# engcang/FAST-LIO-SAM-QN

Measured on AMD Instinct MI355X. Metric: scan-pair registrations/sec on 100k-pt clouds, higher is better.
Workload: dtype f32 search / f64 accumulate

## Files before the change

fast-lio-sam-qn_amd/csrc/qn_gicp_kernels.cuh:

```cuda
#pragma once
#include "qn_device.cuh"
#include "qn_step_math.cuh"
#include "qn_linearize.cuh"
#include "qn_knn_hist.cuh"
#include "../../include/qn_engine.h"
#include "qn_util_kernels.cuh"

namespace qn {

#define QN_ACC_MAX_BLOCKS 512
#define QN_MAX_TRACE 1024

struct GicpState {
  double x0[16], xi[16], delta[16];
  double H[36], b[6], d[6];
  double y0, yi, den;
  double lambda, nu;
  double final_H[36];
  double fitness;
  int outer, inner, phase, converged, lm_failed;
  uint32_t fb_count;
  uint32_t trace_len;
  uint32_t big_count;
  int pending;
  int reserved;
};


__device__ __forceinline__ uint32_t xcd_block(uint32_t b, uint32_t nb) {
  const uint32_t per = nb >> 3, rem = nb & 7u, x = b & 7u;
  return x * per + min(x, rem) + (b >> 3);
}

struct CellCountK {
  static constexpr int TB = QN_BLOCK, OCC = 1;
  struct Args { const float4* pts; uint32_t n; GridView g; uint32_t* counts; uint32_t* cell_of_pt; };
  static __device__ __forceinline__ void run(const Args& a, const uint32_t bx, const uint32_t) {
    const GridView g = grid_resolve(a.g);
    const uint32_t i = bx * QN_BLOCK + threadIdx.x;
    if (i >= a.n) return;
    const float4 p = a.pts[i];
    const int cx = cell_coord(p.x, g.ox, g.inv_cell, g.nx), cy = cell_coord(p.y, g.oy, g.inv_cell, g.ny), cz = cell_coord(p.z, g.oz, g.inv_cell, g.nz);
    const uint32_t c = cell_key(g, cx, cy, cz);
    a.cell_of_pt[i] = c;
    atomicAdd(&a.counts[c], 1u);
  }
};
static __global__ void __launch_bounds__(QN_BLOCK) k_cell_count(const float4* __restrict__ pts, uint32_t n, GridView g, uint32_t* __restrict__ counts, uint32_t* __restrict__ cell_of_pt) {
  const CellCountK::Args a{pts, n, g, counts, cell_of_pt};
  CellCountK::run(a, blockIdx.x, gridDim.x);
}

__device__ inline GridDims grid_dims_from_bbox(const int (&omn)[3], const int (&omx)[3], bool bad, uint32_t n, uint32_t max_cells, double cell_override) {
  GridDims d;
  float mn[3], mx[3];
  for (int a = 0; a < 3; a++) { mn[a] = ord2f(omn[a]); mx[a] = ord2f(omx[a]); }
  bad = bad || !(mx[0] >= mn[0]);
  if (bad) { for (int a = 0; a < 3; a++) { mn[a] = 0.f; mx[a] = 0.f; } }
  double L[3]; for (int a = 0; a < 3; a++) L[a] = fmax((double)mx[a] - (double)mn[a], 0.0);
  const double Lmax = fmax(L[0], fmax(L[1], L[2]));
  const double area = fmax(L[0] * L[1], fmax(L[0] * L[2], L[1] * L[2]));
  double cell = sqrt(4.0 * area / (double)n);
  cell = fmax(cell, fmax(Lmax / 2048.0, 1e-6));
  if (cell_override > 0) cell = cell_override;
  int dims[3] = {1, 1, 1}, tdims[3] = {1, 1, 1}; const int tile[3] = {QN_TX, QN_TY, QN_TZ};
  for (int iter = 0; iter < 64; iter++) {
    double tot = 1;
    for (int a = 0; a < 3; a++) { dims[a] = (int)floor(L[a] / cell) + 1; tdims[a] = (dims[a] + tile[a] - 1) / tile[a]; tot *= (double)tdims[a] * tile[a]; }
    if (tot <= (double)max_cells) break;
    cell *= fmax(cbrt(tot / (double)max_cells), 1.02);
    if (iter == 63) { cell = Lmax + 1.0; for (int a = 0; a < 3; a++) { dims[a] = 1; tdims[a] = 1; } }
  }
  d.ox = mn[0]; d.oy = mn[1]; d.oz = mn[2]; d.cell = (float)cell; d.inv_cell = 1.0f / d.cell;
  d.nx = dims[0]; d.ny = dims[1]; d.nz = dims[2]; d.ntx = tdims[0]; d.nty = tdims[1]; d.ntz = tdims[2];
  float amax = 0; for (int a = 0; a < 3; a++) amax = fmaxf(amax, fmaxf(fabsf(mn[a]), fabsf(mx[a])));
  d.eps = 1e-3f * d.cell + 1e-6f * (amax + (float)Lmax);
  d.n = bad ? 0u : n; d.ncells = (uint32_t)tdims[0] * tdims[1] * tdims[2] * QN_TILE_CELLS; d.nonfinite = bad ? 1u : 0u; d.pad = 0;
  return d;
}

#define QN_BBOX_MAX_BLOCKS 256
struct BBoxAcc { int mn[3], mx[3]; uint32_t nonfinite, ticket; };
struct PackBBoxK {
  static constexpr int TB = QN_BLOCK, OCC = 1;
  struct Args { const char* in; uint32_t stride, n; float4* raw; BBoxAcc* acc; uint32_t max_cells; double cell_override; GridDims* dims_dev; GridDims* dims_host; };
  static __device__ __forceinline__ void run(const Args& a, const uint32_t bx, const uint32_t nbx) {
    __shared__ int smn[QN_BLOCK / 64][3], smx[QN_BLOCK / 64][3], sbad[QN_BLOCK / 64];
    const char* __restrict__ in = a.in; float4* __restrict__ raw = a.raw; BBoxAcc* acc = a.acc;
    const uint32_t n = a.n, stride = a.stride;
    int mn[3] = {0x7fffffff, 0x7fffffff, 0x7fffffff}, mx[3] = {(int)0x80000000, (int)0x80000000, (int)0x80000000};
    int bad = 0;
    for (uint32_t i = bx * QN_BLOCK + threadIdx.x; i < n; i += nbx * QN_BLOCK) {
      const float* q = (const float*)(in + (size_t)i * stride);
      const float4 p = make_float4(q[0], q[1], q[2], 1.0f);
      raw[i] = p;
      if (!(isfinite(p.x) && isfinite(p.y) && isfinite(p.z))) { bad = 1; continue; }
      const int ox = f2ord(p.x), oy = f2ord(p.y), oz = f2ord(p.z);
      mn[0] = min(mn[0], ox); mn[1] = min(mn[1], oy); mn[2] = min(mn[2], oz);
      mx[0] = max(mx[0], ox); mx[1] = max(mx[1], oy); mx[2] = max(mx[2], oz);
    }
#pragma unroll
    for (int d = 0; d < 3; d++) { mn[d] = wave_min_i(mn[d]); mx[d] = wave_max_i(mx[d]); }
    bad = wave_max_i(bad);
    const int wid = threadIdx.x >> 6;
    if ((threadIdx.x & 63) == 0) { for (int d = 0; d < 3; d++) { smn[wid][d] = mn[d]; smx[wid][d] = mx[d]; } sbad[wid] = bad; }
    __syncthreads();
    __shared__ int s_last;
    if (threadIdx.x == 0) {
      for (int w = 1; w < QN_BLOCK / 64; w++) { for (int d = 0; d < 3; d++) { mn[d] = min(mn[d], smn[w][d]); mx[d] = max(mx[d], smx[w][d]); } bad |= sbad[w]; }
      BBoxAcc* mine = acc + 1 + bx;
      for (int d = 0; d < 3; d++) { __hip_atomic_store(&mine->mn[d], mn[d], __ATOMIC_RELAXED, __HIP_MEMORY_SCOPE_AGENT); __hip_atomic_store(&mine->mx[d], mx[d], __ATOMIC_RELAXED, __HIP_MEMORY_SCOPE_AGENT); }
      __hip_atomic_store(&mine->nonfinite, (uint32_t)bad, __ATOMIC_RELAXED, __HIP_MEMORY_SCOPE_AGENT);
      asm volatile("s_waitcnt vmcnt(0)" ::: "memory");
      s_last = __hip_atomic_fetch_add(&acc->ticket, 1u, __ATOMIC_RELAXED, __HIP_MEMORY_SCOPE_AGENT) == nbx - 1u ? 1 : 0;
    }
    __syncthreads();
    if (!s_last) return;
    if (threadIdx.x >= 64) return;
    for (int d = 0; d < 3; d++) { mn[d] = 0x7fffffff; mx[d] = (int)0x80000000; }
    int nf = 0;
    for (uint32_t b = threadIdx.x; b < nbx; b += 64) {
      const BBoxAcc* o = acc + 1 + b;
      for (int d = 0; d < 3; d++) { mn[d] = min(mn[d], __hip_atomic_load(&o->mn[d], __ATOMIC_RELAXED, __HIP_MEMORY_SCOPE_AGENT)); mx[d] = max(mx[d], __hip_atomic_load(&o->mx[d], __ATOMIC_RELAXED, __HIP_MEMORY_SCOPE_AGENT)); }
      nf |= (int)__hip_atomic_load(&o->nonfinite, __ATOMIC_RELAXED, __HIP_MEMORY_SCOPE_AGENT);
    }
#pragma unroll
    for (int d = 0; d < 3; d++) { mn[d] = wave_min_i(mn[d]); mx[d] = wave_max_i(mx[d]); }
    nf = wave_max_i(nf);
    if (threadIdx.x != 0) return;
    const GridDims g = grid_dims_from_bbox(mn, mx, nf != 0, n, a.max_cells, a.cell_override);
    *a.dims_dev = g; *a.dims_host = g;
    __hip_atomic_store(&acc->ticket, 0u, __ATOMIC_RELAXED, __HIP_MEMORY_SCOPE_AGENT);
  }
};
static __global__ void __launch_bounds__(QN_BLOCK) k_pack_bbox_dims(const char* __restrict__ in, uint32_t stride, uint32_t n, float4* __restrict__ raw, BBoxAcc* acc,
                                                                    uint32_t max_cells, double cell_override, GridDims* __restrict__ dims_dev, GridDims* __restrict__ dims_host) {
  const PackBBoxK::Args a{in, stride, n, raw, acc, max_cells, cell_override, dims_dev, dims_host};
  PackBBoxK::run(a, blockIdx.x, gridDim.x);
}
static __global__ void k_bbox_acc_init(BBoxAcc* acc, int count) {
  for (int i = threadIdx.x; blockIdx.x == 0 && i < count; i += blockDim.x) { BBoxAcc a; for (int d = 0; d < 3; d++) { a.mn[d] = 0x7fffffff; a.mx[d] = (int)0x80000000; } a.nonfinite = 0; a.ticket = 0; acc[i] = a; }
}

#define QN_LB_STATE_AGG 1ull
#define QN_LB_STATE_INC 2ull
struct ScanLookbackK {
  static constexpr int TB = QN_BLOCK, OCC = 1;
  struct Args { const uint32_t* in; const GridDims* dims; uint32_t* out; unsigned long long* status; uint32_t epoch, total; };
  static __device__ __forceinline__ void run(const Args& a, const uint32_t bx, const uint32_t) {
    __shared__ uint32_t wsum[QN_BLOCK / 64];
    __shared__ uint32_t s_prefix;
    const uint32_t* __restrict__ in = a.in; uint32_t* __restrict__ out = a.out; unsigned long long* status = a.status;
    const uint32_t total = a.total;
    const uint32_t m = uni(a.dims->ncells);
    const uint32_t tile = bx;
    if (tile * (uint32_t)(QN_BLOCK * QN_SCAN_ITEMS) >= m) return;
// ... 319 lines not shown
  using Args = NnSearchArgs;
  static __device__ __forceinline__ void run(const Args& a, const uint32_t bx, const uint32_t nbx) {
    GridView src = a.src, tgt = a.tgt; const GicpState* __restrict__ st = a.st; const double thr2 = a.thr2; float r0 = a.r0; const int max_rounds = a.max_rounds;
    int32_t* __restrict__ corr = a.corr; float* __restrict__ sqd = a.sqd; int32_t* __restrict__ nn_idx = a.nn_idx; float4* __restrict__ nn_ref = a.nn_ref;
    uint2* __restrict__ fb_list = a.fb_list; uint32_t* __restrict__ fb_count = a.fb_count; uint2* __restrict__ big_list = a.big_list; uint32_t* __restrict__ big_count = a.big_count;
    const int big_blocks = a.big_blocks; const float big_ratio = a.big_ratio; uint32_t* __restrict__ far_stats = a.far_stats; const NnOpt opt = a.opt;

  __shared__ WaveLds lds[BLOCK / 64];
  if (MODE == 0 && uni(st->phase) != 0) return;
  if (MODE == 1 && uni(st->phase) != 2) return;
  if (opt.cond && !(uni(st->reserved) & opt.cond)) return;
  src = grid_resolve(src); tgt = grid_resolve(tgt); if (r0 < 0.f) r0 = -r0 * tgt.cell;
  __shared__ float sTf[12];
  if (threadIdx.x < 12) sTf[threadIdx.x] = (float)st->x0[threadIdx.x];
  __syncthreads();
  if (LIST && (int)bx >= (int)nbx - big_blocks) {
    const uint32_t nbig = uni(*big_count);
    if (tgt.dbg && bx == nbx - 1 && threadIdx.x == 0) atomicAdd(&tgt.dbg[7], nbig);
    uint32_t nfar = 0;
    const uint32_t bw0 = (bx - (nbx - big_blocks)) * (BLOCK / 64) + (threadIdx.x >> 6), nbw = big_blocks * (BLOCK / 64);
    const uint32_t E = (GROUP && opt.group && nbig >= (uint32_t)opt.group_min) ? min(16u, (nbig + (uint32_t)opt.group - 1u) / (uint32_t)opt.group) : 1u;
    if (GROUP && E > 1u) {
      const int lane = threadIdx.x & 63, qs = lane & 15;
      WaveLds* wl = &lds[threadIdx.x >> 6];
      const float INF = __int_as_float(0x7f800000);
      for (uint32_t w0 = bw0 * E; w0 < nbig; w0 += nbw * E) {
        const uint32_t slot = w0 + (uint32_t)qs;
        const bool active = (uint32_t)qs < E && slot < nbig;
        const uint2 rec = active ? big_list[slot] : make_uint2(0u, 0u);
        const float4 p = active ? src.pts[rec.x] : make_float4(0.f, 0.f, 0.f, 0.f);
        float qx, qy, qz; { float Tf[12];
#pragma unroll
          for (int j = 0; j < 12; j++) Tf[j] = sTf[j];
          xform_query<MODE>(Tf, p.x, p.y, p.z, qx, qy, qz); }
        const float v = __uint_as_float(rec.y);
        const float r = v > 0.f ? v * 1.1f + 0.5f * tgt.cell : -v;
        const bool finite_q = (qx - qx == 0.f) && (qy - qy == 0.f) && (qz - qz == 0.f) && (r - r == 0.f);
        unsigned long long key = QN_INF_KEY; float second = INF, d_unseen = INF;
        unsigned long long todo = __ballot(active);
        while (todo) {
          const int al = __ffsll((long long)todo) - 1;
          const float ax = rdlane(qx, al), ay = rdlane(qy, al), az = rdlane(qz, al), ar = rdlane(r, al);
          const bool afin = rdlane((int)finite_q, al) != 0;
          const bool open_q = (todo >> lane) & 1ull;
          const bool member = open_q && (qs == (al & 15) || (afin && finite_q && sqdist(qx, qy, qz, ax, ay, az) <= 0.25f * ar * ar));
          const unsigned long long mm = __ballot(member);
          if (__popcll(mm) <= 4) {
            unsigned long long k1; float s1, du1;
            wave_search_single(tgt, ax, ay, az, ar, INF, k1, s1, du1, wl);
            if (member) { key = k1; second = s1; d_unseen = du1; }
          } else {
            wave_search_far16(tgt, qx, qy, qz, member, r, key, second, d_unseen, wl);
          }
          todo &= ~mm;
        }
        if (active && lane < 16) {
          const uint32_t tl = late(rec.x);
          store_nn<MODE>(key, late(__float_as_uint(p.w)), tl, thr2, corr, sqd, nn_idx);
          if (MODE == 0) nn_ref[tl] = make_float4(qx, qy, qz, key != QN_INF_KEY ? sqrtf(key_d2(key)) : INF);
        }
        if (far_stats && MODE == 0) {
          const unsigned long long fm = __ballot(active && lane < 16 && key != QN_INF_KEY && key_d2(key) > 36.f * tgt.cell * tgt.cell);
          if (lane == 0) nfar += (uint32_t)__popcll(fm);
        }
      }
      if (far_stats && MODE == 0 && (threadIdx.x & 63) == 0 && nfar) atomicAdd(&far_stats[3], nfar);
      return;
    }
    unsigned long long pr_sum = 0, pr_max = 0, pr_a = 0, pr_b = 0; uint32_t pr_n = 0;
    const uint32_t nfb_all = uni(*fb_count);
    const uint32_t nfb1 = (opt.fb_small && nfb_all <= opt.fb_small) ? nfb_all : 0u;
    for (uint32_t w = bw0; w < nbig + nfb1; w += nbw) {
      const uint2 rec = w < nbig ? big_list[w] : fb_list[w - nbig];
      const float4 p = src.pts[rec.x];
      float qx, qy, qz; { float Tf[12];
#pragma unroll
          for (int j = 0; j < 12; j++) Tf[j] = sTf[j];
          xform_query<MODE>(Tf, p.x, p.y, p.z, qx, qy, qz); }
      const float v = __uint_as_float(rec.y);
      const float r = v > 0.f ? v * 1.1f + 0.5f * tgt.cell : -v;
      unsigned long long key; float second, d_unseen;
      const unsigned long long pt0 = opt.probe ? wall_clock64() : 0ull;
      SingleStats sst;
      wave_search_single(tgt, qx, qy, qz, r, __int_as_float(0x7f800000), key, second, d_unseen, &lds[threadIdx.x >> 6], sst, opt.probe != nullptr);
      if (opt.probe) { const unsigned long long dt = wall_clock64() - pt0; pr_sum += dt; pr_n++;
        if (dt > pr_max) { pr_max = dt; pr_a = ((unsigned long long)sst.rounds << 48) | ((unsigned long long)min(sst.segs, 0xffffffu) << 24) | (unsigned long long)min(sst.cand, 0xffffffu);
          pr_b = ((unsigned long long)__float_as_uint(sst.r_first) << 32) | __float_as_uint(key != QN_INF_KEY ? sqrtf(key_d2(key)) : -1.f); } }
      if ((threadIdx.x & 63) == 0) {
        const uint32_t tl = late(rec.x);
        store_nn<MODE>(key, late(__float_as_uint(p.w)), tl, thr2, corr, sqd, nn_idx);
        if (MODE == 0) nn_ref[tl] = make_float4(qx, qy, qz, fminf(sqrtf(second), d_unseen));
        if (key != QN_INF_KEY && key_d2(key) > 36.f * tgt.cell * tgt.cell) nfar++;
      }
    }
    if (far_stats && MODE == 0 && (threadIdx.x & 63) == 0 && nfar) atomicAdd(&far_stats[3], nfar);
    if (opt.probe && (threadIdx.x & 63) == 0 && bw0 < 16384u) { opt.probe[4 * bw0] = (pr_max << 32) | pr_n; opt.probe[4 * bw0 + 1] = pr_sum; opt.probe[4 * bw0 + 2] = pr_a; opt.probe[4 * bw0 + 3] = pr_b; }
    return;
  }
  const uint32_t nq = LIST ? uni(*fb_count) : src.n;
  if (LIST && opt.fb_small && nq <= opt.fb_small) return;
  if (LIST && tgt.dbg && bx == 0 && threadIdx.x == 0) atomicAdd(&tgt.dbg[5], nq);
  const uint32_t wave0 = bx * (BLOCK / 64) + (threadIdx.x >> 6), nwaves = (nbx - (LIST ? big_blocks : 0)) * (BLOCK / 64);
  for (uint32_t base = wave0 * 16; base < nq; base += nwaves * 16) {
    const uint32_t slot = base + (threadIdx.x & 15);
    const bool active = slot < nq;
    uint32_t t = slot; float r = r0, r_cap = __int_as_float(0x7f800000);
    if (LIST && active) {
      const uint2 rec = fb_list[slot]; t = rec.x;
      const float v = __uint_as_float(rec.y);
      if (v < 0.f) r = -v; else { r_cap = v; r = fminf(v, r0); }
    }
    const float4 p = active ? src.pts[t] : make_float4(0, 0, 0, 0);
    float qx, qy, qz; { float Tf[12];
#pragma unroll
          for (int j = 0; j < 12; j++) Tf[j] = sTf[j];
          xform_query<MODE>(Tf, p.x, p.y, p.z, qx, qy, qz); }
    Best1 sink; sink.init();
    float d_unseen;
    const bool cert = wave_search<4>(tgt, qx, qy, qz, active, r, r_cap, max_rounds, sink, &lds[threadIdx.x >> 6], d_unseen);
    const bool mine = active && (threadIdx.x & 48) == 0;
    const bool done = cert || LIST;
    if (!LIST && MODE == 0 && opt.clear_ref && mine) opt.clear_ref[t] = make_float4(0.f, 0.f, 0.f, 0.f);
    if (mine && done) {
      const uint32_t tl = late(t);
      store_nn<MODE>(sink.key, late(__float_as_uint(p.w)), tl, thr2, corr, sqd, nn_idx);
      if (MODE == 0) nn_ref[tl] = make_float4(qx, qy, qz, fminf(sqrtf(sink.second), d_unseen));
    }
    if (!LIST) {
      const float rn = r;
      const bool far = rn > big_ratio * r0;
      wave_append(big_list, big_count, mine && !done && far, make_uint2(t, __float_as_uint(-rn)));
      wave_append(fb_list, fb_count, mine && !done && !far, make_uint2(t, __float_as_uint(-rn)));
    }
  }
  }
};
template <int MODE, bool LIST, int BLOCK, bool GROUP = false>
__global__ void __launch_bounds__(BLOCK, GROUP ? 5 : 6) k_nn_search(GridView src, GridView tgt, const GicpState* __restrict__ st, double thr2, float r0, int max_rounds,
                                                        int32_t* __restrict__ corr, float* __restrict__ sqd, int32_t* __restrict__ nn_idx, float4* __restrict__ nn_ref,
                                                        uint2* __restrict__ fb_list, uint32_t* __restrict__ fb_count,
                                                        uint2* __restrict__ big_list, uint32_t* __restrict__ big_count, int big_blocks, float big_ratio, uint32_t* __restrict__ far_stats, NnOpt opt) {
  const NnSearchArgs a{src, tgt, st, thr2, r0, max_rounds, corr, sqd, nn_idx, nn_ref, fb_list, fb_count, big_list, big_count, big_blocks, big_ratio, far_stats, opt};
  NnSearchK<MODE, LIST, BLOCK, GROUP>::run(a, blockIdx.x, gridDim.x);
}


typedef __attribute__((address_space(1))) unsigned long long qn_gu64;
__device__ __forceinline__ void pr_store(unsigned long long* p, unsigned long long bits) { __hip_atomic_store((qn_gu64*)p, bits, __ATOMIC_RELAXED, __HIP_MEMORY_SCOPE_AGENT); }
__device__ __forceinline__ unsigned long long pr_load(const unsigned long long* p) { return __hip_atomic_load((qn_gu64*)p, __ATOMIC_RELAXED, __HIP_MEMORY_SCOPE_AGENT); }
__device__ __forceinline__ void row_store(double* p, double v, const bool coherent) {
  if (coherent) pr_store((unsigned long long*)p, (unsigned long long)__double_as_longlong(v)); else *p = v;
}

#define QN_LANE_ROWS 9
template <int MODE>
struct NnLaneK {
  static constexpr int TB = 256, OCC = 6;
  using Args = NnSearchArgs;
  static __device__ __forceinline__ void run(const Args& a, const uint32_t bx, const uint32_t) {
    const GicpState* __restrict__ st = a.st; const NnOpt opt = a.opt;
    if (MODE == 0 && uni(st->phase) != 0) return;
    if (MODE == 1 && uni(st->phase) != 2) return;
    if (opt.cond && !(uni(st->reserved) & opt.cond)) return;
    const GridView src = grid_resolve(a.src), tgt = grid_resolve(a.tgt);
    float r0 = a.r0; if (r0 < 0.f) r0 = -r0 * tgt.cell;
    float Tf[12];
#pragma unroll
    for (int j = 0; j < 12; j++) Tf[j] = uni((float)st->x0[j]);
    const uint32_t t = bx * TB + threadIdx.x;
    const bool active = t < src.n;
    const float4 p = active ? src.pts[t] : make_float4(0, 0, 0, 0);
    float qx, qy, qz; xform_query<MODE>(Tf, p.x, p.y, p.z, qx, qy, qz);
    if (MODE == 0 && opt.clear_ref && active) opt.clear_ref[t] = make_float4(0.f, 0.f, 0.f, 0.f);
    float r = r0;
    const int x0 = cell_coord(qx - r, tgt.ox, tgt.inv_cell, tgt.nx), x1 = cell_coord(qx + r, tgt.ox, tgt.inv_cell, tgt.nx);
    const int y0 = cell_coord(qy - r, tgt.oy, tgt.inv_cell, tgt.ny), y1 = cell_coord(qy + r, tgt.oy, tgt.inv_cell, tgt.ny);
    const int z0 = cell_coord(qz - r, tgt.oz, tgt.inv_cell, tgt.nz), z1 = cell_coord(qz + r, tgt.oz, tgt.inv_cell, tgt.nz);
    const int tx0 = x0 >> 3, ntr = (x1 >> 3) - tx0 + 1, nyr = y1 - y0 + 1, nzr = z1 - z0 + 1;
    const bool scan = active && nyr <= 3 && nzr <= 3 && ntr <= 2;
    Best1 sink; sink.init();
    const float4* __restrict__ pts = tgt.pts; const uint32_t* __restrict__ cs = tgt.cell_start;
    const uint32_t tile_zy = (uint32_t)tgt.nty * (uint32_t)tgt.ntx;
    uint32_t kz[3], ky[3];
#pragma unroll
    for (int d = 0; d < 3; d++) {
      const int z = z0 + d, y = y0 + d;
      kz[d] = (((uint32_t)(z >> 2) * tile_zy) << 7) | ((uint32_t)(z & 3) << 5);
      ky[d] = (((uint32_t)(y >> 2) * (uint32_t)tgt.ntx) << 7) | ((uint32_t)(y & 3) << 3);
    }
    const bool two = scan && ntr == 2;
    const int xb0 = min(x1, (tx0 << 3) + 7);
    const uint32_t kx0 = ((uint32_t)tx0 << 7) | (uint32_t)(x0 & 7), xlen0 = (uint32_t)(xb0 - x0) + 1u;
    const uint32_t kx1 = (uint32_t)(tx0 + 1) << 7, xlen1 = (uint32_t)(x1 - ((tx0 + 1) << 3)) + 1u;
    uint32_t s0[QN_LANE_ROWS], len0[QN_LANE_ROWS], off1[QN_LANE_ROWS], tot[QN_LANE_ROWS];
#pragma unroll
    for (int rr = 0; rr < QN_LANE_ROWS; rr++) {
      const int dz = rr / 3, dy = rr % 3;
      const bool rv = scan && dy < nyr && dz < nzr;
      uint32_t a0 = 0, b0 = 0, a1 = 0, b1 = 0;
      const uint32_t kr = kz[dz] + ky[dy];
      if (rv) { a0 = cs[kr + kx0]; b0 = cs[kr + kx0 + xlen0]; }
      if (rv && two) { a1 = cs[kr + kx1]; b1 = cs[kr + kx1 + xlen1]; }
      s0[rr] = a0; len0[rr] = b0 - a0; off1[rr] = a1 - len0[rr]; tot[rr] = len0[rr] + (b1 - a1);
    }
#pragma unroll
    for (int rr = 0; rr < QN_LANE_ROWS; rr++) {
      const uint32_t l0 = len0[rr], sa = s0[rr], sb = off1[rr], last = tot[rr] - 1u;
      for (uint32_t v = 0; v < tot[rr]; v += 4) {
        const uint32_t v1 = min(v + 1u, last), v2 = min(v + 2u, last), v3 = min(v + 3u, last);
        const float4 c0 = pts[v + (v < l0 ? sa : sb)], c1 = pts[v1 + (v1 < l0 ? sa : sb)], c2 = pts[v2 + (v2 < l0 ? sa : sb)], c3 = pts[v3 + (v3 < l0 ? sa : sb)];
        sink.consider<true>(true, sqdist(qx, qy, qz, c0.x, c0.y, c0.z), __float_as_uint(c0.w));
        sink.consider<true>(v + 1u <= last, sqdist(qx, qy, qz, c1.x, c1.y, c1.z), __float_as_uint(c1.w));
        sink.consider<true>(v + 2u <= last, sqdist(qx, qy, qz, c2.x, c2.y, c2.z), __float_as_uint(c2.w));
        sink.consider<true>(v + 3u <= last, sqdist(qx, qy, qz, c3.x, c3.y, c3.z), __float_as_uint(c3.w));
      }
    }
    const float INF = __int_as_float(0x7f800000);
    bool certified = false; float d_unseen = INF;
    if (scan) {
      float d = INF;
      if (x0 > 0) d = fminf(d, qx - (tgt.ox + x0 * tgt.cell));
      if (x1 < tgt.nx - 1) d = fminf(d, (tgt.ox + (x1 + 1) * tgt.cell) - qx);
      if (y0 > 0) d = fminf(d, qy - (tgt.oy + y0 * tgt.cell));
      if (y1 < tgt.ny - 1) d = fminf(d, (tgt.oy + (y1 + 1) * tgt.cell) - qy);
      if (z0 > 0) d = fminf(d, qz - (tgt.oz + z0 * tgt.cell));
      if (z1 < tgt.nz - 1) d = fminf(d, (tgt.oz + (z1 + 1) * tgt.cell) - qz);
      if (d == INF || !(r == r)) { certified = true; d_unseen = INF; }
      else { d -= tgt.eps; d_unseen = d; certified = d > 0.f && sink.full() && sink.worst_d2() < d * d; }
      if (!certified) r = sink.full() ? fmaxf(sqrtf(sink.worst_d2()) * 1.000001f + tgt.eps, r + tgt.eps) : 2.f * r + tgt.cell;
    }
    if (active && certified) {
      store_nn<MODE>(sink.key, __float_as_uint(p.w), t, a.thr2, a.corr, a.sqd, a.nn_idx);
      if (MODE == 0) a.nn_ref[t] = make_float4(qx, qy, qz, fminf(sqrtf(sink.second), d_unseen));
    }
    const bool far = r > a.big_ratio * r0;
    wave_append(a.big_list, a.big_count, active && !certified && far, make_uint2(t, __float_as_uint(-r)));
    wave_append(a.fb_list, a.fb_count, active && !certified && !far, make_uint2(t, __float_as_uint(-r)));
  }
};
template <int MODE>
__global__ void __launch_bounds__(256, 6) k_nn_lane(NnSearchArgs a) { NnLaneK<MODE>::run(a, blockIdx.x, gridDim.x); }


#define QN_TRACK_SEG 8
__device__ __forceinline__ bool track_bound_holds(float d0, float delta, float bound) {
  return (sqrtf(d0) + delta) * 1.000004f < bound;
}
template <int MODE>
__global__ void __launch_bounds__(QN_BLOCK, 6) k_nn_track(GridView src, GridView tgt, const float4* __restrict__ tgt_raw, const GicpState* __restrict__ st,
                                                       double thr2, int32_t* __restrict__ corr, float* __restrict__ sqd, int32_t* __restrict__ nn_idx,
                                                       float4* __restrict__ nn_ref, uint2* __restrict__ fb_list, uint32_t* __restrict__ fb_count,
                                                       uint2* __restrict__ big_list, uint32_t* __restrict__ big_count) {
  if (MODE == 0 && st->phase != 0) return;
  if (MODE == 1 && st->phase != 2) return;
  src = grid_resolve(src); tgt = grid_resolve(tgt);
  float Tf[12];
#pragma unroll
  for (int j = 0; j < 12; j++) Tf[j] = (float)st->x0[j];
  const uint32_t lblk = xcd_block(blockIdx.x, gridDim.x);
  const uint32_t t = lblk * QN_BLOCK + threadIdx.x;
  if (t >= src.n) return;
  const float INF = __int_as_float(0x7f800000);
  const float4 p = src.pts[t];
  const uint32_t i = __float_as_uint(p.w);
  float qx, qy, qz; xform_query<MODE>(Tf, p.x, p.y, p.z, qx, qy, qz);
  unsigned long long best = QN_INF_KEY; float second = INF, d_unseen = INF;
  bool rescanned = false, big = false, noseed = false;
  float r = 0.f, delta = 0.f;
  const bool finite_q = (qx - qx == 0.f) && (qy - qy == 0.f) && (qz - qz == 0.f);
  const uint32_t j0 = (uint32_t)nn_idx[t];
  if (finite_q && j0 >= tgt.n) { noseed = true; big = true; r = tgt.cell; }
  if (finite_q && !noseed) {
    const float4 ref = nn_ref[t];
    const float4 p0 = tgt_raw[j0];
    const float d0 = sqdist(qx, qy, qz, p0.x, p0.y, p0.z);
    best = pack_key(d0, j0);
    delta = sqrtf(sqdist(qx, qy, qz, ref.x, ref.y, ref.z));
    if (track_bound_holds(d0, delta, ref.w)) {
      if (tgt.dbg && (threadIdx.x & 63) == 0) atomicAdd(&tgt.dbg[6], (uint32_t)__popcll(__ballot(1)));
    } else {
      r = sqrtf(d0) * 1.000001f + tgt.eps;
      const int bx0 = cell_coord(qx - r, tgt.ox, tgt.inv_cell, tgt.nx), bx1 = cell_coord(qx + r, tgt.ox, tgt.inv_cell, tgt.nx);
      const int by0 = cell_coord(qy - r, tgt.oy, tgt.inv_cell, tgt.ny), by1 = cell_coord(qy + r, tgt.oy, tgt.inv_cell, tgt.ny);
      const int bz0 = cell_coord(qz - r, tgt.oz, tgt.inv_cell, tgt.nz), bz1 = cell_coord(qz + r, tgt.oz, tgt.inv_cell, tgt.nz);
      const int tx0 = bx0 >> 3, ntr = (bx1 >> 3) - tx0 + 1, nyr = by1 - by0 + 1;
      const int nseg = ntr * nyr * (bz1 - bz0 + 1);
      if (!(d0 == d0) || nseg > QN_TRACK_SEG) big = true;
      else {
        uint32_t s[QN_TRACK_SEG], e[QN_TRACK_SEG];
#pragma unroll
        for (int sg = 0; sg < QN_TRACK_SEG; sg++) {
          s[sg] = 0; e[sg] = 0;
          if (sg < nseg) {
            int tt, rr; divmod_small(sg, ntr, rr, tt);
            int qz_, ry_; divmod_small(rr, nyr, qz_, ry_);
            const int ry = by0 + ry_, rz = bz0 + qz_, tx = tx0 + tt;
            const int xa = max(bx0, tx << 3), xb = min(bx1, (tx << 3) + 7);
            const uint32_t k0 = cell_key(tgt, xa, ry, rz);
            s[sg] = tgt.cell_start[k0]; e[sg] = tgt.cell_start[k0 + (xb - xa) + 1];
          }
        }
#pragma unroll
        for (int sg = 0; sg < QN_TRACK_SEG; sg++) {
          for (uint32_t u = s[sg]; u < e[sg]; u++) {
            const float4 a = tgt.pts[u];
            const float da = sqdist(qx, qy, qz, a.x, a.y, a.z);
            const unsigned long long ka = pack_key(da, __float_as_uint(a.w));
            if (ka < best) { second = key_d2(best); best = ka; }
            else if (ka != best && da < second) second = da;
          }
        }
        float d = INF;
        if (bx0 > 0) d = fminf(d, qx - (tgt.ox + bx0 * tgt.cell));
        if (bx1 < tgt.nx - 1) d = fminf(d, (tgt.ox + (bx1 + 1) * tgt.cell) - qx);
        if (by0 > 0) d = fminf(d, qy - (tgt.oy + by0 * tgt.cell));
        if (by1 < tgt.ny - 1) d = fminf(d, (tgt.oy + (by1 + 1) * tgt.cell) - qy);
        if (bz0 > 0) d = fminf(d, qz - (tgt.oz + bz0 * tgt.cell));
        if (bz1 < tgt.nz - 1) d = fminf(d, (tgt.oz + (bz1 + 1) * tgt.cell) - qz);
        d_unseen = d - tgt.eps; rescanned = true;
      }
    }
  }
  const bool tight_far = r > 2.5f * tgt.cell && delta < 0.25f * r;
  wave_append(big_list, big_count, big && tight_far, make_uint2(t, __float_as_uint(r)));
  wave_append(fb_list, fb_count, big && !tight_far, make_uint2(t, __float_as_uint(noseed ? -r : r)));
  if (big) return;
  store_nn<MODE>(best, i, t, thr2, corr, sqd, nn_idx);
  if (MODE == 0 && rescanned) nn_ref[t] = make_float4(qx, qy, qz, fminf(sqrtf(second), d_unseen));
}

static __global__ void k_reset_lists(GicpState* st) { if (threadIdx.x == 0 && blockIdx.x == 0) { st->fb_count = 0; st->big_count = 0; } }
static __global__ void k_verify_nn(uint32_t n, const GicpState* __restrict__ st, const int32_t* __restrict__ nn_a, const int32_t* __restrict__ nn_b,
                                   const float* __restrict__ sqd_a, const float* __restrict__ sqd_b, const int32_t* __restrict__ corr_a, const int32_t* __restrict__ corr_b,
                                   uint32_t* __restrict__ counters ) {
  if (st->phase != 0) return;
  const uint32_t t = blockIdx.x * blockDim.x + threadIdx.x;
  if (t == 0) atomicAdd(&counters[1], 1u);
  if (t >= n) return;
  bool bad = nn_a[t] != nn_b[t];
  if (sqd_a) bad = bad || __float_as_uint(sqd_a[t]) != __float_as_uint(sqd_b[t]) || corr_a[t] != corr_b[t];
  if (bad) { atomicAdd(&counters[0], 1u); atomicCAS(&counters[2], 0u, t + 1u); }
}


__device__ __forceinline__ void d_propose(GicpState* st, double lambda, SolveWork* A) {
  double Hl[36], rhs[6], dl[6];
#pragma unroll
  for (int i = 0; i < 6; i++)
#pragma unroll
    for (int j = 0; j < 6; j++) Hl[6 * i + j] = j <= i ? st->H[6 * i + j] : 0.0;
  if (!d_ldlt_solve6_fast(Hl, lambda, rhs, dl, st->b)) {
#pragma unroll
    for (int i = 0; i < 6; i++) A->rhs[i] = rhs[i];
    d_ldlt_solve6(st->H, lambda, st->d, A);
#pragma unroll
    for (int i = 0; i < 6; i++) dl[i] = st->d[i];
  }
  double R[3][3]; d_so3_exp(dl, R);
  double delta[16], xi[16];
#pragma unroll
  for (int i = 0; i < 16; i++) delta[i] = 0;
#pragma unroll
  for (int a = 0; a < 3; a++) {
#pragma unroll
    for (int b = 0; b < 3; b++) delta[4 * a + b] = R[a][b];
    delta[4 * a + 3] = dl[3 + a];
  }
// ... 316 lines not shown
```

Baseline: 4496.

## Flatten per-lane cell-row walk into a single queue-driven trip loop

Replaces the nested loop over nine cell rows, each with its own variable trip count, with a per-lane work queue in shared memory. A single flattened loop then runs for the wave-maximum total trip count, so lanes with short rows pick up their next row and do not idle while others finish long rows. This targets wavefront divergence from uneven row lengths. It costs shared memory (about 27 KB per block), extra queue bookkeeping, and a fallback pass that re-reads cell starts for rows too large to pack into 16 bits.

```diff
diff --git a/fast-lio-sam-qn_amd/csrc/qn_gicp_kernels.cuh b/fast-lio-sam-qn_amd/csrc/qn_gicp_kernels.cuh
--- a/fast-lio-sam-qn_amd/csrc/qn_gicp_kernels.cuh
+++ b/fast-lio-sam-qn_amd/csrc/qn_gicp_kernels.cuh
@@ -2,6 +2,7 @@
 #include "qn_device.cuh"
 #include "qn_step_math.cuh"
 #include "qn_linearize.cuh"
+#include "qn_lane_walk.cuh"
 #include "qn_knn_hist.cuh"
 #include "../../include/qn_engine.h"
 #include "qn_util_kernels.cuh"
@@ -627,11 +628,19 @@
   if (coherent) pr_store((unsigned long long*)p, (unsigned long long)__double_as_longlong(v)); else *p = v;
 }
 
-#define QN_LANE_ROWS 9
 template <int MODE>
 struct NnLaneK {
   static constexpr int TB = 256, OCC = 6;
   using Args = NnSearchArgs;
+  static __device__ __forceinline__ void lane_trip(Best1& sink, const float4* __restrict__ pts, const float qx, const float qy, const float qz,
+                                                   const uint32_t v, const uint32_t l0, const uint32_t sa, const uint32_t sb, const uint32_t last) {
+    const uint32_t v1 = min(v + 1u, last), v2 = min(v + 2u, last), v3 = min(v + 3u, last);
+    const float4 c0 = pts[v + (v < l0 ? sa : sb)], c1 = pts[v1 + (v1 < l0 ? sa : sb)], c2 = pts[v2 + (v2 < l0 ? sa : sb)], c3 = pts[v3 + (v3 < l0 ? sa : sb)];
+    sink.consider<true>(true, sqdist(qx, qy, qz, c0.x, c0.y, c0.z), __float_as_uint(c0.w));
+    sink.consider<true>(v + 1u <= last, sqdist(qx, qy, qz, c1.x, c1.y, c1.z), __float_as_uint(c1.w));
+    sink.consider<true>(v + 2u <= last, sqdist(qx, qy, qz, c2.x, c2.y, c2.z), __float_as_uint(c2.w));
+    sink.consider<true>(v + 3u <= last, sqdist(qx, qy, qz, c3.x, c3.y, c3.z), __float_as_uint(c3.w));
+  }
   static __device__ __forceinline__ void run(const Args& a, const uint32_t bx, const uint32_t) {
     const GicpState* __restrict__ st = a.st; const NnOpt opt = a.opt;
     if (MODE == 0 && uni(st->phase) != 0) return;
@@ -678,16 +687,30 @@
       if (rv && two) { a1 = cs[kr + kx1]; b1 = cs[kr + kx1 + xlen1]; }
       s0[rr] = a0; len0[rr] = b0 - a0; off1[rr] = a1 - len0[rr]; tot[rr] = len0[rr] + (b1 - a1);
     }
+    __shared__ uint32_t lane_q[QN_LANE_QUEUE * 3 * TB];
+    uint32_t* const q = &lane_q[threadIdx.x];
+    LaneWalk<TB> w; w.init();
+    bool wide = false;
 #pragma unroll
     for (int rr = 0; rr < QN_LANE_ROWS; rr++) {
-      const uint32_t l0 = len0[rr], sa = s0[rr], sb = off1[rr], last = tot[rr] - 1u;
-      for (uint32_t v = 0; v < tot[rr]; v += 4) {
-        const uint32_t v1 = min(v + 1u, last), v2 = min(v + 2u, last), v3 = min(v + 3u, last);
-        const float4 c0 = pts[v + (v < l0 ? sa : sb)], c1 = pts[v1 + (v1 < l0 ? sa : sb)], c2 = pts[v2 + (v2 < l0 ? sa : sb)], c3 = pts[v3 + (v3 < l0 ? sa : sb)];
-        sink.consider<true>(true, sqdist(qx, qy, qz, c0.x, c0.y, c0.z), __float_as_uint(c0.w));
-        sink.consider<true>(v + 1u <= last, sqdist(qx, qy, qz, c1.x, c1.y, c1.z), __float_as_uint(c1.w));
-        sink.consider<true>(v + 2u <= last, sqdist(qx, qy, qz, c2.x, c2.y, c2.z), __float_as_uint(c2.w));
-        sink.consider<true>(v + 3u <= last, sqdist(qx, qy, qz, c3.x, c3.y, c3.z), __float_as_uint(c3.w));
+      const LaneRow row{s0[rr], off1[rr], len0[rr], tot[rr]};
+      wide |= !(rr < QN_LANE_QUEUE ? w.push(q, row) : w.seed(row));
+    }
+    const int ntrip = wave_max_i((int)w.trips);
+    for (int trip = 0; trip < ntrip; trip++) {
+      if (w.next(q)) { lane_trip(sink, pts, qx, qy, qz, w.v, w.len0, w.s0, w.off1, w.tot - 1u); w.step(); }
+    }
+    if (__any(wide)) {
+#pragma unroll
+      for (int rr = 0; rr < QN_LANE_ROWS; rr++) {
+        const int dz = rr / 3, dy = rr % 3;
+        const bool rv = scan && dy < nyr && dz < nzr;
+        uint32_t a0 = 0, b0 = 0, a1 = 0, b1 = 0;
+        const uint32_t kr = kz[dz] + ky[dy];
+        if (rv) { a0 = cs[kr + kx0]; b0 = cs[kr + kx0 + xlen0]; }
+        if (rv && two) { a1 = cs[kr + kx1]; b1 = cs[kr + kx1 + xlen1]; }
+        const uint32_t l0 = b0 - a0, sb = a1 - l0, n = l0 + (b1 - a1);
+        if (!lane_row_fits(n)) for (uint32_t v = 0; v < n; v += 4) lane_trip(sink, pts, qx, qy, qz, v, l0, a0, sb, n - 1u);
       }
     }
     const float INF = __int_as_float(0x7f800000);
diff --git a/fast-lio-sam-qn_amd/csrc/qn_lane_walk.cuh b/fast-lio-sam-qn_amd/csrc/qn_lane_walk.cuh
--- /dev/null
+++ b/fast-lio-sam-qn_amd/csrc/qn_lane_walk.cuh
@@ -0,0 +1,47 @@
+#pragma once
+#include <cstdint>
+#if defined(__HIPCC__)
+#define QN_LW_FN __host__ __device__ __forceinline__
+#else
+#define QN_LW_FN inline
+#endif
+#define QN_LANE_ROWS 9
+#define QN_LANE_QUEUE (QN_LANE_ROWS - 1)
+#define QN_LANE_ROW_MAX 0xffffu
+
+struct LaneRow { uint32_t s0, off1, len0, tot; };
+
+QN_LW_FN uint32_t lane_row_trips(const uint32_t tot) { return (tot + 3u) >> 2; }
+QN_LW_FN bool lane_row_fits(const uint32_t tot) { return tot <= QN_LANE_ROW_MAX; }
+
+template <int STRIDE>
+struct LaneWalk {
+  uint32_t s0, off1, len0, tot, v;
+  uint32_t head, tail;
+  uint32_t trips;
+  QN_LW_FN void init() { s0 = off1 = len0 = tot = v = head = tail = trips = 0u; }
+  QN_LW_FN bool push(uint32_t* q, const LaneRow& r) {
+    if (!lane_row_fits(r.tot)) return false;
+    if (r.tot != 0u) {
+      q[tail] = r.s0; q[tail + STRIDE] = r.off1; q[tail + 2 * STRIDE] = r.len0 | (r.tot << 16);
+      tail += 3u * STRIDE; trips += lane_row_trips(r.tot);
+    }
+    return true;
+  }
+  QN_LW_FN bool seed(const LaneRow& r) {
+    if (!lane_row_fits(r.tot)) return false;
+    s0 = r.s0; off1 = r.off1; len0 = r.len0; tot = r.tot; v = 0u; trips += lane_row_trips(r.tot);
+    return true;
+  }
+  QN_LW_FN bool next(const uint32_t* q) {
+    if (v >= tot && head < tail) {
+      const uint32_t lens = q[head + 2 * STRIDE];
+      s0 = q[head]; off1 = q[head + STRIDE]; len0 = lens & 0xffffu; tot = lens >> 16; v = 0u;
+      head += 3u * STRIDE;
+    }
+    return v < tot;
+  }
+  QN_LW_FN uint32_t count() const { return tot - v < 4u ? tot - v : 4u; }
+  QN_LW_FN uint32_t at(const uint32_t u) const { return u + (u < len0 ? s0 : off1); }
+  QN_LW_FN void step() { v += 4u; }
+};
```

After: 4535 (median of 5 runs). Within noise of the previous version (+0.9%).
